# QEDProtocol/city-rollup

Measured on AMD Instinct MI355X. Metric: ms/NTT at 2^20 Goldilocks (commit-shaped step: 135-column 2^20-row NTT + Poseidon Merkle cap), lower is better.
Workload: dtype u64 (Goldilocks mod 2^64-2^32+1; the Poseidon MDS layers are evaluated exactly on 32-bit limbs held in f64); 1 GPU; configs[1]: 2^20-row x 135-column trace, forward NTT per column (natural->bit-reversed) + Poseidon Merkle cap height 4; log_n=20, columns=135, cap_height=4

## Files before the change

### city-rollup_amd/csrc/cityprover.hip

```cpp
#include "core.h"
#include "merkle.h"
#include "ntt.h"
#include "ntt16.h"
#include "poseidon.h"
#include "poseidon_coop.h"

namespace {

int get_pow_table(cp_ctx *ctx, uint64_t base, const uint64_t **out) {
  auto it = ctx->pow_tables.find(base);
  if (it != ctx->pow_tables.end()) {
    *out = it->second.get<uint64_t>();
    return CP_OK;
  }
  std::vector<uint64_t> h(3 * ntt::PT_SIZE);
  uint64_t b = base;
  for (int lvl = 0; lvl < 3; lvl++) {
    uint64_t acc = 1;
    for (int j = 0; j < ntt::PT_SIZE; j++) {
      h[lvl * ntt::PT_SIZE + j] = acc;
      acc = gl::mul(acc, b);
    }
    b = acc;
  }
  DevBuf t = ctx->buf();
  CP_TRY(alloc_status(ctx, t.alloc(h.size() * sizeof(uint64_t)), h.size() * sizeof(uint64_t)));
  HIP_TRY(ctx, hipMemcpyAsync(t.get(), h.data(), h.size() * sizeof(uint64_t), hipMemcpyHostToDevice, ctx->stream));
  HIP_TRY(ctx, hipStreamSynchronize(ctx->stream));
  *out = t.get<uint64_t>();
  ctx->pow_tables[base] = std::move(t);
  return CP_OK;
}

uint64_t root_of_unity(int log_n, bool inverse) {
  return inverse ? GL_ROOTS_INV[log_n] : GL_ROOTS[log_n];
}

int get_prescale_table(cp_ctx *ctx, int log_n, int rate_bits, uint64_t shift, const uint64_t **out) {
  cp_ctx::PreKey key{log_n, rate_bits, shift};
  auto it = ctx->prescale_tables.find(key);
  if (it != ctx->prescale_tables.end()) {
    *out = it->second.get<uint64_t>();
    return CP_OK;
  }
  const uint64_t *stab, *wtabN;
  CP_TRY(get_pow_table(ctx, shift, &stab));
  CP_TRY(get_pow_table(ctx, root_of_unity(log_n + rate_bits, false), &wtabN));
  size_t N = (size_t)1 << (log_n + rate_bits);
  DevBuf T = ctx->buf();
  CP_TRY(alloc_status(ctx, T.alloc(N * sizeof(uint64_t)), N * sizeof(uint64_t)));
  LAUNCH(ctx, "lde_fill_prescale", ntt16::k_fill_prescale, dim3((unsigned)((N + 255) / 256)), dim3(256), T.get<uint64_t>(),
         log_n, rate_bits, stab, wtabN);
  *out = T.get<uint64_t>();
  ctx->prescale_tables[key] = std::move(T);
  return CP_OK;
}

}
namespace quot {
__global__ __launch_bounds__(256) void k_fill_l0(uint64_t *out, size_t N, int log_N, int rb, const uint64_t *omega_tab, const uint64_t *zh,
                                                 uint64_t n_field);
}
namespace {

int get_l0_table(cp_ctx *ctx, int log_n, int rate_bits, const uint64_t *omega_tab, const uint64_t *zh, const uint64_t **out) {
  auto it = ctx->l0_tables.find({log_n, rate_bits});
  if (it == ctx->l0_tables.end()) {
    const size_t N = (size_t)1 << (log_n + rate_bits);
    DevBuf tab = ctx->buf();
    CP_TRY(alloc_status(ctx, tab.alloc(N * 8), N * 8));
    LAUNCH(ctx, "quotient_fill_l0", quot::k_fill_l0, dim3(blocks_for(N, 256)), dim3(256), tab.get<uint64_t>(), N, log_n + rate_bits, rate_bits,
           omega_tab, zh, ((uint64_t)1 << log_n) % gl::P);
    HIP_TRY(ctx, sync_stream(ctx));
    it = ctx->l0_tables.emplace(std::make_pair(log_n, rate_bits), std::move(tab)).first;
  }
  *out = it->second.get<uint64_t>();
  return CP_OK;
}

__global__ void k_self_test(const uint64_t *__restrict__ a, const uint64_t *__restrict__ b, uint64_t *__restrict__ out, int n_mul) {
  const int i = threadIdx.x;
  if (i < n_mul) out[i] = gl::mul(a[i], b[i]);
  if (i == 63) {
    uint64_t s[poseidon::W];
    for (int k = 0; k < poseidon::W; k++) s[k] = a[k];
    poseidon::permute(s);
    for (int k = 0; k < poseidon::W; k++) out[n_mul + k] = s[k];
  }
}
int power_on_self_test(cp_ctx *ctx) {
  constexpr int N = 16;
  const uint64_t M = ~0ull, P = gl::P;
  const uint64_t a[N] = {0, 1, P - 1, P - 1, M, M, 1ull << 48, 0xFFFFFFFFull << 32, 0x123456789ABCDEF1ull, 0xFFFFFFFF00000000ull,
                         0x8000000080000000ull, 0xFFFFFFFEFFFFFFFFull, 0xdeadbeefull << 32, 0x9E3779B97F4A7C15ull, 3, P + 5};
  const uint64_t b[N] = {M, M, P - 1, 2, M, P, 3ull << 48, 0xFFFFFFFFull << 32, 0xF0E1D2C3B4A59687ull, 0xFFFFFFFF00000001ull,
                         0x8000000080000000ull, 0xFFFFFFFEFFFFFFFFull, 0xfeedfaceull << 32, 0xD1B54A32D192ED03ull, M / 3, M - 7};
  uint64_t want[N + poseidon::W], got[N + poseidon::W];
  for (int i = 0; i < N; i++) want[i] = gl::mul(a[i], b[i]);
  {
    uint64_t s[poseidon::W];
    for (int k = 0; k < poseidon::W; k++) s[k] = a[k];
    poseidon::permute_host(s);
    for (int k = 0; k < poseidon::W; k++) want[N + k] = s[k];
  }
  CP_TRY(ensure_scratch(ctx, (3 * N + poseidon::W) * sizeof(uint64_t)));
  uint64_t *da = ctx->scratch.get<uint64_t>(), *db = da + N, *dout = db + N;
  CP_TRY(cp_h2d(ctx, da, a, sizeof a));
  CP_TRY(cp_h2d(ctx, db, b, sizeof b));
  LAUNCH(ctx, "self_test", k_self_test, dim3(1), dim3(64), da, db, dout, N);
  CP_TRY(cp_d2h(ctx, got, dout, sizeof got));
  if (hostu::fault_fires(CP_FAULT_SELFTEST)) got[7] ^= 1;
  for (int i = 0; i < N + poseidon::W; i++)
    if (got[i] != want[i])
      return set_error(ctx, CP_ERR_INTERNAL, "device arithmetic self-test failed (%s %d): this GPU does not execute the field kernels correctly",
                       i < N ? "product" : "permutation word", i < N ? i : i - N);
  return CP_OK;
}

int upload_constants(cp_ctx *ctx) {
  HIP_TRY(ctx, hipMemcpyToSymbol(HIP_SYMBOL(poseidon::d_RC), POSEIDON_RC, sizeof POSEIDON_RC));
  HIP_TRY(ctx, hipMemcpyToSymbol(HIP_SYMBOL(poseidon::d_RCD), POSEIDON_RCD, sizeof POSEIDON_RCD));
  HIP_TRY(ctx, hipMemcpyToSymbol(HIP_SYMBOL(poseidon::d_DDK), poseidon::DDK_HOST, sizeof poseidon::DDK_HOST));
  HIP_TRY(ctx, hipMemcpyToSymbol(HIP_SYMBOL(poseidon::d_DDLAST), poseidon::DDLAST_HOST, sizeof poseidon::DDLAST_HOST));
  return CP_OK;
}



struct DifExtra {
  const uint64_t *src = nullptr;
  size_t src_stride = 0;
  const uint64_t *ptab = nullptr;
  size_t block_stride = 0;
  int n_blocks = 1, block_bits = 0;
  bool natural_out = false;
};

int run_dif(cp_ctx *ctx, uint64_t *data, int log_n, size_t batch, size_t stride, bool inverse,
            uint64_t scale, const uint64_t *stab_pre, const DifExtra &ex = DifExtra()) {
  if (log_n == 0) return CP_OK;
  const uint64_t *wtab;
  CP_TRY(get_pow_table(ctx, root_of_unity(log_n, inverse), &wtab));
  int q = log_n;
  bool first = true;
  while (q > 0) {
    int L, c;
    int remaining = q;
    if (remaining <= ntt::LOG_TILE_MAX) {
      L = remaining;
    } else {
      int front = remaining - ntt::LOG_TILE_MAX;
      if (front >= 4 && front <= ntt::LOG_TILE_MAX - 4) L = front;
      else {
        int passes = (remaining + 9) / 10;
        L = (remaining + passes - 1) / passes;
      }
    }
    int q_after = q - L;
    c = ntt::LOG_TILE_MAX - L;
    int outer_bits = log_n - L;
    if (c > outer_bits) c = outer_bits;
    if (q_after > 0 && c > q_after) c = q_after;
    ntt::PassArgs a;
    a.data = data;
    a.stride = stride;
    a.wtab = wtab;
    a.stab = stab_pre;
    a.log_n = log_n;
    a.q = q_after;
    a.L = L;
    a.c = c;
    a.first = first;
    a.last = (q_after == 0);
    a.scale = scale;
    a.coset_pre = stab_pre != nullptr;
    a.coset_post = 0;
    a.src = ex.src;
    a.src_stride = ex.src_stride;
    a.ptab = ex.ptab;
    a.block_stride = ex.block_stride;
    a.block_bits = ex.block_bits;
    a.natural_out = ex.natural_out ? 1 : 0;
    const int staged = (int)CP_KNOB(ctx, "NTT_STAGED_STORE", 1);
    a.staged_store = (staged && q_after == 0 && log_n >= 16) ? 1 : 0;
    dim3 grid((unsigned)(((size_t)1 << outer_bits) >> c), (unsigned)batch, (unsigned)ex.n_blocks);
    bool done = false;
    const bool need16 = ex.src || ex.ptab || ex.n_blocks > 1 || ex.natural_out;
    static const bool ntt_v1 = getenv("CITYPROVER_NTT_V1") != nullptr;
    if (L >= 4 && L + c == ntt16::LOG_TILE && (need16 || !ntt_v1)) {
      const bool half = log_n >= 16;
#define PASS16_(LL, ROWS_, NAME)                                                                                              \
  if (inverse) {                                                                                                              \
    if (half) LAUNCH(ctx, NAME, (ntt16::k_dif_pass16<LL, 12 - LL, ROWS_, true, true>), grid, dim3(ntt16::THREADS), a);        \
    else LAUNCH(ctx, NAME, (ntt16::k_dif_pass16<LL, 12 - LL, ROWS_, true, false>), grid, dim3(ntt16::THREADS), a);            \
  } else {                                                                                                                    \
    if (half) LAUNCH(ctx, NAME, (ntt16::k_dif_pass16<LL, 12 - LL, ROWS_, false, true>), grid, dim3(ntt16::THREADS), a);       \
    else LAUNCH(ctx, NAME, (ntt16::k_dif_pass16<LL, 12 - LL, ROWS_, false, false>), grid, dim3(ntt16::THREADS), a);           \
  }
#define PASS16(LL)                                 \
  case LL:                                         \
    if (q_after == 0) {                            \
      PASS16_(LL, true, "ntt16_rows")              \
    } else {                                       \
      PASS16_(LL, false, "ntt16_cols")             \
    }                                              \
    done = true;                                   \
    break;
      switch (L) {
        PASS16(4) PASS16(5) PASS16(6) PASS16(7) PASS16(8) PASS16(9) PASS16(10) PASS16(11) PASS16(12)
        default: break;
      }
#undef PASS16
#undef PASS16_
    }
    if (!done && need16) return set_error(ctx, CP_ERR_INTERNAL, "radix-16 pass required but unavailable (L=%d c=%d)", L, c);
    if (!done) {
      if (q_after == 0)
        LAUNCH(ctx, "ntt_dif_pass_rows", ntt::k_dif_pass<true>, grid, dim3(ntt::THREADS), a);
      else
        LAUNCH(ctx, "ntt_dif_pass_cols", ntt::k_dif_pass<false>, grid, dim3(ntt::THREADS), a);
    }
    q = q_after;
    first = false;
  }
  return CP_OK;
}

int bitrev_copy(cp_ctx *ctx, const uint64_t *src, uint64_t *dst, size_t src_stride,
                size_t dst_stride, int log_n, size_t batch, const uint64_t *stab) {
  size_t n = (size_t)1 << log_n;
  dim3 grid(blocks_for(n, 256), (unsigned)batch);
  LAUNCH(ctx, "ntt_bitrev_copy", ntt::k_bitrev_copy, grid, dim3(256), src, dst, src_stride, dst_stride,
         log_n, stab);
  return CP_OK;
}

size_t merkle_words_per_tree(size_t n_leaves, int cap_height) {
  size_t cap_n = (size_t)1 << cap_height;
  size_t nodes = n_leaves > cap_n ? 2 * n_leaves - 2 * cap_n : n_leaves;
  return nodes * 4;
}

int merkle_fuse_levels(cp_ctx *ctx) {
  const int v = (int)CP_KNOB(ctx, "MERKLE_FUSE", 1);
  return v < 0 ? 0 : v > 3 ? 3 : v;
}
int merkle_level_fuse_levels(cp_ctx *ctx) {
  const int v = (int)CP_KNOB(ctx, "MERKLE_LEVEL_FUSE", 0);
  return v < 0 ? 0 : v > 3 ? 3 : v;
}
int fusable_levels(size_t nodes, size_t cap_n, int want) {
  if (nodes % merkle::THREADS) return 0;
  int f = 0;
  while (f < want && (nodes >> (f + 1)) > cap_n) f++;
  return f;
}

int merkle_levels(cp_ctx *ctx, uint64_t *D, size_t per_tree, size_t n_leaves, size_t n_trees,
                  int cap_height, uint64_t *caps, int done = 0) {
  size_t cap_n = (size_t)1 << cap_height;
  size_t n = n_leaves, off = 0;
  for (int l = 0; l < done; l++, n >>= 1) off += n * 4;
  while (n > cap_n) {
    size_t np = n / 2;
    const uint64_t *child = D + off;
    uint64_t *parent;
    size_t pstride;
    if (np == cap_n) { parent = caps; pstride = cap_n * 4; }
    else { parent = D + off + n * 4; pstride = per_tree; }
    const size_t coop_max = (size_t)CP_KNOB(ctx, "COOP_MAX", 16384);
    const int fuse_max = (int)CP_KNOB(ctx, "COOP_FUSE", pcoop::MAX_FUSED);
    if (np * n_trees <= coop_max && fuse_max >= 1) {
      while (n > cap_n) {
        int levels = 0;
        while (levels < fuse_max && levels < pcoop::MAX_FUSED && (n >> levels) > cap_n) levels++;
        const unsigned waves = ((1u << (levels - 1)) + pcoop::STATES_PER_WAVE - 1) / pcoop::STATES_PER_WAVE;
        LAUNCH(ctx, "merkle_levels_coop", pcoop::k_levels_coop, dim3((unsigned)(n >> levels), (unsigned)n_trees), dim3(64 * waves), D, off, n,
               levels, per_tree, caps, cap_n);
        for (int l = 0; l < levels; l++, n >>= 1) off += n * 4;
      }
      break;
    }
    int fuse = np == cap_n ? 0 : fusable_levels(np, cap_n, merkle_level_fuse_levels(ctx));
    while (fuse > 0 && (np >> fuse) * n_trees < coop_max) fuse--;
    if (fuse > 0) {
      const dim3 g((unsigned)(np / merkle::THREADS), (unsigned)n_trees), b(merkle::THREADS);
      if (fuse == 1) LAUNCH(ctx, "merkle_level_fused", merkle::k_level_fused<1>, g, b, D, off, np, per_tree);
      else if (fuse == 2) LAUNCH(ctx, "merkle_level_fused", merkle::k_level_fused<2>, g, b, D, off, np, per_tree);
      else LAUNCH(ctx, "merkle_level_fused", merkle::k_level_fused<3>, g, b, D, off, np, per_tree);
      for (int l = 0; l <= fuse; l++, n >>= 1) off += n * 4;
      continue;
    }
    if (np * n_trees <= coop_max)
      LAUNCH(ctx, "merkle_level_coop", pcoop::k_level_coop, dim3(blocks_for(np, pcoop::STATES_PER_BLOCK), (unsigned)n_trees), dim3(256), child,
             np, parent, per_tree, pstride);
    else
      LAUNCH(ctx, "merkle_level", merkle::k_level, dim3(blocks_for(np, merkle::THREADS), (unsigned)n_trees),
             dim3(merkle::THREADS), child, np, parent, per_tree, pstride);
    off += n * 4;
    n = np;
  }
  if (n_leaves == cap_n) {
    HIP_TRY(ctx, hipMemcpy2DAsync(caps, cap_n * 32, D, per_tree * 8, cap_n * 32, n_trees,
                                  hipMemcpyDeviceToDevice, ctx->stream));
  }
  return CP_OK;
}

int merkle_cols_batch(cp_ctx *ctx, const uint64_t *cols, size_t n_leaves, size_t leaf_len,
                      size_t col_stride, size_t n_trees, size_t tree_cols_stride, int cap_height,
                      uint64_t *digests, uint64_t *caps, const uint64_t *salt = nullptr, int n_salt = 0,
                      size_t salt_tree_stride = 0) {
  size_t per_tree = merkle_words_per_tree(n_leaves, cap_height);
  uint64_t *D = digests;
  if (!D) {
    CP_TRY(ensure_scratch(ctx, n_trees * per_tree * sizeof(uint64_t)));
    D = ctx->scratch.get<uint64_t>();
  }
  const dim3 grid(blocks_for(n_leaves, merkle::THREADS), (unsigned)n_trees), block(merkle::THREADS);
  const size_t coop_leaf_max = (size_t)CP_KNOB(ctx, "COOP_LEAF_MAX", 8192);
  const bool salted = salt && n_salt > 0;
  if (n_leaves * n_trees <= coop_leaf_max && leaf_len + (salted ? (size_t)n_salt : 0) > 4) {
    const dim3 cgrid(blocks_for(n_leaves, pcoop::STATES_PER_BLOCK), (unsigned)n_trees);
    if (salted)
      LAUNCH(ctx, "leaf_hash_cols_coop", pcoop::k_leaf_hash_cols_coop<true>, cgrid, dim3(256), cols, n_leaves, (int)leaf_len, col_stride, D,
             tree_cols_stride, per_tree, salt, n_salt, salt_tree_stride);
    else
      LAUNCH(ctx, "leaf_hash_cols_coop", pcoop::k_leaf_hash_cols_coop<false>, cgrid, dim3(256), cols, n_leaves, (int)leaf_len, col_stride, D,
             tree_cols_stride, per_tree, (const uint64_t *)nullptr, 0, (size_t)0);
    return merkle_levels(ctx, D, per_tree, n_leaves, n_trees, cap_height, caps);
  }
  const size_t coop_max = (size_t)CP_KNOB(ctx, "COOP_MAX", 16384);
  int fuse = fusable_levels(n_leaves, (size_t)1 << cap_height, merkle_fuse_levels(ctx));
  while (fuse > 0 && (n_leaves >> fuse) * n_trees < coop_max) fuse--;
#define CP_LEAF_LAUNCH(SALTED, F, SP, NS, SS)                                                                                          \
  LAUNCH(ctx, "leaf_hash_cols", (merkle::k_leaf_hash_cols<SALTED, F>), grid, block, cols, n_leaves, (int)leaf_len, col_stride, D, \
         tree_cols_stride, per_tree, SP, NS, SS)
  if (salted) {
    if (fuse == 3) CP_LEAF_LAUNCH(true, 3, salt, n_salt, salt_tree_stride);
    else if (fuse == 2) CP_LEAF_LAUNCH(true, 2, salt, n_salt, salt_tree_stride);
    else if (fuse == 1) CP_LEAF_LAUNCH(true, 1, salt, n_salt, salt_tree_stride);
    else CP_LEAF_LAUNCH(true, 0, salt, n_salt, salt_tree_stride);
  } else {
    if (fuse == 3) CP_LEAF_LAUNCH(false, 3, (const uint64_t *)nullptr, 0, (size_t)0);
    else if (fuse == 2) CP_LEAF_LAUNCH(false, 2, (const uint64_t *)nullptr, 0, (size_t)0);
    else if (fuse == 1) CP_LEAF_LAUNCH(false, 1, (const uint64_t *)nullptr, 0, (size_t)0);
    else CP_LEAF_LAUNCH(false, 0, (const uint64_t *)nullptr, 0, (size_t)0);
  }
#undef CP_LEAF_LAUNCH
  return merkle_levels(ctx, D, per_tree, n_leaves, n_trees, cap_height, caps, fuse);
}

bool valid_merkle_shape(size_t n_leaves, int cap_height) {
  if (n_leaves == 0 || (n_leaves & (n_leaves - 1))) return false;
  if (cap_height < 0 || cap_height > 40) return false;
  return ((size_t)1 << cap_height) <= n_leaves;
}

}

namespace { void batches_orphan(cp_ctx *ctx); }

extern "C" {

int cp_abi_version(void) { return CP_ABI_VERSION; }

int cp_fault_inject(int kind, long after) {
  if (kind != CP_FAULT_THREAD && kind != CP_FAULT_ALLOC && kind != CP_FAULT_SELFTEST && kind != CP_FAULT_DEVMEM) return set_error(nullptr, CP_ERR_INVALID_ARG, "unknown fault kind %d", kind);
  hostu::fault_counter(kind).store(after < 0 ? -1 : after);
  return CP_OK;
}

int cp_device_count(void) {
  int n = 0;
  if (hipGetDeviceCount(&n) != hipSuccess) return 0;
  return n;
}

const char *cp_last_error(cp_ctx *ctx) { return ctx ? ctx->error.c_str() : g_tls_error.c_str(); }

cp_ctx *cp_ctx_create(int device) try {
  int n = cp_device_count();
  if (n <= 0) {
    set_error(nullptr, CP_ERR_NO_DEVICE,
              "no HIP device visible: libcityprover_hip has no CPU fallback");
    return nullptr;
  }
  if (device < 0 || device >= n) {
    set_error(nullptr, CP_ERR_INVALID_ARG, "device %d out of range (have %d)", device, n);
    return nullptr;
  }
  cp_ctx *ctx = new (std::nothrow) cp_ctx(device);
  if (!ctx) {
    set_error(nullptr, CP_ERR_OOM, "out of host memory");
    return nullptr;
  }
  auto fail = [&](const char *what, hipError_t e) {
    set_error(nullptr, CP_ERR_HIP, "%s: %s", what, hipGetErrorString(e));
    delete ctx;
    return (cp_ctx *)nullptr;
  };
  hipError_t e = hipSetDevice(device);
  if (e != hipSuccess) return fail("hipSetDevice", e);
  e = hipStreamCreateWithFlags(&ctx->stream, hipStreamNonBlocking);
  if (e != hipSuccess) return fail("hipStreamCreate", e);
  if (upload_constants(ctx) != CP_OK || power_on_self_test(ctx) != CP_OK) {
    std::string msg = ctx->error;
    cp_ctx_destroy(ctx);
    g_tls_error = msg;
    return nullptr;
  }
  return ctx;
} catch (...) {
  exception_status(nullptr);
  return nullptr;
}

void cp_ctx_destroy(cp_ctx *ctx) {
  if (!ctx) return;
  batches_orphan(ctx);
  for (cp_ctx *lane : ctx->lanes) cp_ctx_destroy(lane);
  ctx->lanes.clear();
  hipSetDevice(ctx->device);
  if (ctx->stream) hipStreamSynchronize(ctx->stream);
  prof_flush(ctx);
  for (auto e : ctx->prof_pool) hipEventDestroy(e);
  ctx->pow_tables.clear(); ctx->prescale_tables.clear(); ctx->l0_tables.clear(); ctx->air_sel_tables.clear(); ctx->fr_twiddles.clear();
  ctx->arena.chunks.clear();
  for (DevBuf *b : {&ctx->scratch, &ctx->wires_stage, &ctx->fr_work, &ctx->fr_pow[0].tab, &ctx->fr_pow[1].tab, &ctx->msm_ws,
                     &ctx->fixed_base[0].tab, &ctx->fixed_base[1].tab}) b->reset();
  ctx->pin.reset();
  ctx->noncanonical_flag.reset();
  if (ctx->stream) hipStreamDestroy(ctx->stream);
  delete ctx;
}

int cp_ctx_set_lanes(cp_ctx *ctx, int lanes) try {
  CHECK_CTX(ctx);
  if (ctx->parent) return set_error(ctx, CP_ERR_INVALID_ARG, "a lane has no lanes of its own");
  if (lanes < 1 || lanes > 8) return set_error(ctx, CP_ERR_INVALID_ARG, "lanes must be 1..8 (got %d)", lanes);
  while ((int)ctx->lanes.size() < lanes) {
    cp_ctx *lane = cp_ctx_create(ctx->device);
    if (!lane) return lane_error(ctx);
    lane->parent = ctx;
    lane->transcript_mode = ctx->transcript_mode;
    ctx->lanes.push_back(lane);
  }
  ctx->n_lanes = lanes;
  return CP_OK;
} CP_CATCH(ctx)

int cp_ctx_set_option(cp_ctx *ctx, const char *name, long value) try {
  CHECK_CTX(ctx);
  if (!name) return set_error(ctx, CP_ERR_INVALID_ARG, "NULL argument");
  if (ctx->parent) return set_error(ctx, CP_ERR_INVALID_ARG, "a lane takes its options from its parent");
  bool known = false;
  for (const char *const *k = knob_names(); *k; k++) known = known || strcmp(*k, name) == 0;
  if (!known) return set_error(ctx, CP_ERR_INVALID_ARG, "unknown option \"%s\" (see INTEGRATION.md section 5b)", name);
  for (auto &kv : ctx->options)
    if (kv.first == name) { kv.second = value; return CP_OK; }
  ctx->options.emplace_back(name, value);
  return CP_OK;
} CP_CATCH(ctx)

int cp_ctx_set_device_transcript(cp_ctx *ctx, int mode) try {
  CHECK_CTX(ctx);
  if (mode < -1 || mode > 1) return set_error(ctx, CP_ERR_INVALID_ARG, "mode must be -1 (automatic), 0 (host) or 1 (device)");
  ctx->transcript_mode = mode;
  for (cp_ctx *l : ctx->lanes) l->transcript_mode = mode;
  return CP_OK;
} CP_CATCH(ctx)

int cp_dev_alloc(cp_ctx *ctx, size_t bytes, void **out) try {
  CHECK_CTX(ctx);
  if (!out) return set_error(ctx, CP_ERR_INVALID_ARG, "out is NULL");
  *out = nullptr;
  if (bytes == 0) return CP_OK;
  DevBuf b = ctx->buf();
  CP_TRY(alloc_status(ctx, b.alloc(bytes), bytes));
  *out = b.release();
  return CP_OK;
} CP_CATCH(ctx)
int cp_dev_free(cp_ctx *ctx, void *ptr) try {
  CHECK_CTX(ctx);
  if (!ptr) return CP_OK;
  HIP_TRY(ctx, hipStreamSynchronize(ctx->stream));
  HIP_TRY(ctx, abi_dev_free(ptr));
  return CP_OK;
} CP_CATCH(ctx)
int cp_host_alloc(cp_ctx *ctx, size_t bytes, void **out) try {
  CHECK_CTX(ctx);
  if (!out) return set_error(ctx, CP_ERR_INVALID_ARG, "out is NULL");
  *out = nullptr;
  if (bytes == 0) return CP_OK;
  PinBuf b(pin_pool(), ctx->device);
  CP_TRY(alloc_status(ctx, b.alloc(bytes), bytes));
  *out = b.release();
  return CP_OK;
} CP_CATCH(ctx)
int cp_host_free(cp_ctx *ctx, void *ptr) try {
  CHECK_CTX(ctx);
  if (!ptr) return CP_OK;
  HIP_TRY(ctx, hipStreamSynchronize(ctx->stream));
  HIP_TRY(ctx, abi_host_free(ptr));
  return CP_OK;
} CP_CATCH(ctx)
int cp_h2d(cp_ctx *ctx, void *dst, const void *src, size_t bytes) try {
  CHECK_CTX(ctx);
  if (bytes == 0) return CP_OK;
  if (!dst || !src) return set_error(ctx, CP_ERR_INVALID_ARG, "NULL pointer");
  HIP_TRY(ctx, hipMemcpyAsync(dst, src, bytes, hipMemcpyHostToDevice, ctx->stream));
// ... 422 lines not shown
```

### city-rollup_amd/csrc/ntt.h

```cpp
#pragma once
#include "gl.h"

namespace ntt {

constexpr int LOG_TILE_MAX = 12;
constexpr int TILE_MAX = 1 << LOG_TILE_MAX;
constexpr int THREADS = 256;
constexpr int PT_BITS = 11;
constexpr int PT_SIZE = 1 << PT_BITS;

__device__ __forceinline__ uint64_t pow_table(const uint64_t *__restrict__ T, uint64_t e) {
  uint32_t e0 = (uint32_t)e & (PT_SIZE - 1), e1 = (uint32_t)(e >> PT_BITS) & (PT_SIZE - 1),
           e2 = (uint32_t)(e >> (2 * PT_BITS));
  uint64_t r = T[e0];
  if (e1) r = gl::mul(r, T[PT_SIZE + e1]);
  if (e2) r = gl::mul(r, T[2 * PT_SIZE + e2]);
  return r;
}

__device__ __forceinline__ uint32_t bitrev(uint32_t x, int bits) {
  return bits ? (__brev(x) >> (32 - bits)) : 0;
}

struct PassArgs {
  uint64_t *data;
  size_t stride;
  const uint64_t *wtab;
  const uint64_t *stab;
  int log_n;
  int q, L, c;
  int first, last;
  uint64_t scale;
  int coset_pre;
  int coset_post;
  const uint64_t *src;
  size_t src_stride;
  const uint64_t *ptab;
  size_t block_stride;
  int block_bits;
  int natural_out;
  int staged_store;
};

template <bool ROWS_CONTIG>
__device__ __forceinline__ int lds_pos(int r, int cc, int L, int c) {
  return ROWS_CONTIG ? (cc << L) + r : (r << c) + cc;
}

template <bool ROWS_CONTIG>
__global__ __launch_bounds__(THREADS) void k_dif_pass(PassArgs a) {
  __shared__ uint64_t tile[TILE_MAX];
  __shared__ uint64_t ltw[TILE_MAX / 2];
  const int L = a.L, c = a.c, q = a.q;
  const int tile_elems = 1 << (L + c);
  const int tid = threadIdx.x;
  uint64_t *poly = a.data + (size_t)blockIdx.y * a.stride;
  const uint32_t o_base = blockIdx.x << c;
  const uint32_t qmask = (1u << q) - 1;

  for (int e = tid; e < (1 << (L - 1)); e += THREADS)
    ltw[e] = pow_table(a.wtab, (uint64_t)e << (a.log_n - L));

  for (int p = tid; p < tile_elems; p += THREADS) {
    int r, cc;
    if (ROWS_CONTIG) { cc = p >> L; r = p & ((1 << L) - 1); }
    else { r = p >> c; cc = p & ((1 << c) - 1); }
    uint32_t o = o_base + cc;
    size_t idx = ((size_t)(o >> q) << (q + L)) | ((size_t)r << q) | (o & qmask);
    uint64_t v = poly[idx];
    if (a.coset_pre && a.first) v = gl::mul(v, pow_table(a.stab, idx));
    tile[p] = v;
  }
  __syncthreads();

  const int n_bfly = tile_elems >> 1;
  for (int t = 0; t < L; t++) {
    const int hb = L - 1 - t;
    const int half = 1 << hb;
    for (int b = tid; b < n_bfly; b += THREADS) {
      int cc, pr;
      if (ROWS_CONTIG) { cc = b >> (L - 1); pr = b & ((1 << (L - 1)) - 1); }
      else { pr = b >> c; cc = b & ((1 << c) - 1); }
      int j = pr & (half - 1);
      int r0 = ((pr >> hb) << (hb + 1)) | j;
      int p0 = lds_pos<ROWS_CONTIG>(r0, cc, L, c), p1 = lds_pos<ROWS_CONTIG>(r0 + half, cc, L, c);
      uint64_t u = tile[p0], v = tile[p1];
      tile[p0] = gl::add(u, v);
      tile[p1] = gl::mul(gl::sub(u, v), ltw[j << t]);
    }
    __syncthreads();
  }

  for (int p = tid; p < tile_elems; p += THREADS) {
    int r, cc;
    if (ROWS_CONTIG) { cc = p >> L; r = p & ((1 << L) - 1); }
    else { r = p >> c; cc = p & ((1 << c) - 1); }
    uint32_t o = o_base + cc;
    uint32_t lo = o & qmask;
    size_t idx = ((size_t)(o >> q) << (q + L)) | ((size_t)r << q) | lo;
    uint64_t v = tile[p];
    if (q > 0) {
      uint64_t e = (uint64_t)lo * bitrev(r, L);
      if (e) v = gl::mul(v, pow_table(a.wtab, e << (a.log_n - q - L)));
    }
    if (a.last && a.scale) v = gl::mul(v, a.scale);
    poly[idx] = v;
  }
}

__global__ void k_bitrev_copy(const uint64_t *__restrict__ src, uint64_t *__restrict__ dst,
                              size_t src_stride, size_t dst_stride, int log_n,
                              const uint64_t *__restrict__ stab) {
  size_t i = (size_t)blockIdx.x * blockDim.x + threadIdx.x;
  if (i >> log_n) return;
  const uint64_t *s = src + (size_t)blockIdx.y * src_stride;
  uint64_t *d = dst + (size_t)blockIdx.y * dst_stride;
  uint64_t v = s[bitrev((uint32_t)i, log_n)];
  if (stab) v = gl::mul(v, pow_table(stab, i));
  d[i] = v;
}

__global__ void k_pad_copy(const uint64_t *__restrict__ src, uint64_t *__restrict__ dst,
                           size_t src_stride, size_t dst_stride, size_t n, size_t N) {
  size_t i = (size_t)blockIdx.x * blockDim.x + threadIdx.x;
  if (i >= N) return;
  dst[(size_t)blockIdx.y * dst_stride + i] = i < n ? src[(size_t)blockIdx.y * src_stride + i] : 0;
}

}
```

### city-rollup_amd/csrc/ntt16.h

```cpp
#pragma once
#include <type_traits>

#include "gl.h"
#include "ntt.h"

namespace ntt16 {

template <int K>
GL_HD uint64_t mul_pow2(uint64_t x) {
  static_assert(K >= 0 && K < 96, "shift out of range");
  if constexpr (K == 0) {
    return x;
  } else if constexpr (K < 64) {
    return gl::reduce128(x << K, x >> (64 - K));
  } else {
    constexpr int J = K - 64;
    uint64_t y0 = J ? (x << J) : x;
    uint64_t y1 = J ? (x >> (64 - J)) : 0;
    uint64_t t = gl::reduce128(0, y0);
    return gl::sub(t, y1 << 32);
  }
}

template <bool INV, int E>
GL_HD uint64_t diff_times_w16(uint64_t u, uint64_t v) {
  constexpr int SH = ((INV ? 36 : 156) * (E & 15)) % 192;
  constexpr bool NEG = SH >= 96;
  constexpr int K = SH % 96;
  uint64_t d = NEG ? gl::sub(v, u) : gl::sub(u, v);
  return mul_pow2<K>(d);
}

template <bool INV, int B, bool UNIT_T>
GL_HD void stage(uint64_t (&x)[16], uint64_t T) {
#pragma unroll
  for (int m = 0; m < 16; m++) {
    if (m & (1 << B)) continue;
    const int i = m & ((1 << B) - 1);
    uint64_t u = x[m], v = x[m + (1 << B)];
    x[m] = gl::add(u, v);
    uint64_t d;
    switch (i << (3 - B)) {
      case 0: d = diff_times_w16<INV, 0>(u, v); break;
      case 1: d = diff_times_w16<INV, 1>(u, v); break;
      case 2: d = diff_times_w16<INV, 2>(u, v); break;
      case 3: d = diff_times_w16<INV, 3>(u, v); break;
      case 4: d = diff_times_w16<INV, 4>(u, v); break;
      case 5: d = diff_times_w16<INV, 5>(u, v); break;
      case 6: d = diff_times_w16<INV, 6>(u, v); break;
      default: d = diff_times_w16<INV, 7>(u, v); break;
    }
    x[m + (1 << B)] = UNIT_T ? d : gl::mul(d, T);
  }
}

#if defined(NTT16_SINGLE_CHAINS) || defined(NTT16_STAGE_TWIDDLES)
#define NTT16_PAIRS 0
#else
#define NTT16_PAIRS 1
#endif

template <int K0, int K1>
GL_HD void mul_pow2_2(uint64_t &x, uint64_t &y) {
  static_assert(K0 > 0 && K0 < 96 && K1 > 0 && K1 < 96 && (K0 < 64) == (K1 < 64), "two shifts of one form");
  if constexpr (K0 < 64) {
    gl::reduce128_2(x << K0, x >> (64 - K0), y << K1, y >> (64 - K1), x, y);
  } else {
    constexpr int J0 = K0 - 64, J1 = K1 - 64;
    const uint64_t x0 = J0 ? (x << J0) : x, x1 = J0 ? (x >> (64 - J0)) : 0;
    const uint64_t y0 = J1 ? (y << J1) : y, y1 = J1 ? (y >> (64 - J1)) : 0;
    uint64_t t, u;
    gl::reduce128_2(0, x0, 0, y0, t, u);
    x = gl::sub(t, x1 << 32);
    y = gl::sub(u, y1 << 32);
  }
}

template <bool INV>
constexpr int w16_shift(int E) { return ((INV ? 36 : 156) * (E & 15)) % 192; }

struct ShiftPlan {
  int a[8], b[8], n;
};
template <bool INV, int B>
constexpr ShiftPlan shift_plan() {
  ShiftPlan p{};
  int pend[2] = {-1, -1};
  for (int m = 0; m < 16; m++) {
    if (m & (1 << B)) continue;
    const int K = w16_shift<INV>((m & ((1 << B) - 1)) << (3 - B)) % 96;
    if (K == 0) continue;
    const int form = K >= 64, reg = m + (1 << B);
    if (pend[form] < 0) {
      pend[form] = reg;
    } else {
      p.a[p.n] = pend[form];
      p.b[p.n++] = reg;
      pend[form] = -1;
    }
  }
  for (int form = 0; form < 2; form++)
    if (pend[form] >= 0) {
      p.a[p.n] = pend[form];
      p.b[p.n++] = -1;
    }
  return p;
}
template <bool INV, int B>
constexpr int reg_shift(int reg) { return w16_shift<INV>((reg & ((1 << B) - 1)) << (3 - B)) % 96; }

template <bool INV, int B, int I = 0>
GL_HD void apply_shifts(uint64_t (&x)[16]) {
  constexpr ShiftPlan p = shift_plan<INV, B>();
  if constexpr (I < p.n) {
    constexpr int ra = p.a[I], rb = p.b[I];
    if constexpr (rb < 0) x[ra] = mul_pow2<reg_shift<INV, B>(ra)>(x[ra]);
    else mul_pow2_2<reg_shift<INV, B>(ra), reg_shift<INV, B>(rb)>(x[ra], x[rb]);
    apply_shifts<INV, B, I + 1>(x);
  }
}

template <bool INV, int B>
GL_HD void stage_pairs(uint64_t (&x)[16]) {
#pragma unroll
  for (int m = 0; m < 16; m++) {
    if (m & (1 << B)) continue;
    const bool neg = w16_shift<INV>((m & ((1 << B) - 1)) << (3 - B)) >= 96;
    const uint64_t u = x[m], v = x[m + (1 << B)];
    x[m] = gl::add(u, v);
    x[m + (1 << B)] = neg ? gl::sub(v, u) : gl::sub(u, v);
  }
  apply_shifts<INV, B>(x);
}

constexpr int round_exp(int NSTAGES, int m) {
  int em = 0;
  for (int B = 3; B >= 4 - NSTAGES; B--) em += ((m >> B) & 1) << (3 - B);
  return em;
}
constexpr int round_reg(int NSTAGES, int E, int K) {
  for (int m = 0; m < 16; m++)
    if (round_exp(NSTAGES, m) == E && K-- == 0) return m;
  return -1;
}
template <int NSTAGES, int E, int K>
GL_HD void apply_power(uint64_t (&x)[16], uint64_t pw) {
  constexpr int CNT = 16 >> NSTAGES;
  if constexpr (K + 1 < CNT) {
    constexpr int m0 = round_reg(NSTAGES, E, K), m1 = round_reg(NSTAGES, E, K + 1);
    gl::mul2(x[m0], pw, x[m1], pw, x[m0], x[m1]);
    apply_power<NSTAGES, E, K + 2>(x, pw);
  } else if constexpr (K < CNT) {
    constexpr int m0 = round_reg(NSTAGES, E, K);
    x[m0] = gl::mul(x[m0], pw);
  }
}
template <int NSTAGES, int E = 1>
GL_HD void walk_powers(uint64_t (&x)[16], uint64_t pw, uint64_t T3) {
  constexpr int LAST = (1 << NSTAGES) - 1;
  if constexpr (E < LAST) {
    constexpr int m0 = round_reg(NSTAGES, E, 0);
    uint64_t next, r;
    gl::mul_lazy2(pw, T3, x[m0], pw, next, r);
    x[m0] = gl::canon(r);
    apply_power<NSTAGES, E, 1>(x, pw);
    walk_powers<NSTAGES, E + 1>(x, next, T3);
  } else {
    apply_power<NSTAGES, E, 0>(x, pw);
  }
}

template <bool INV, int NSTAGES, bool UNIT_T>
GL_HD void round16(uint64_t (&x)[16], uint64_t T3) {
#if defined(NTT16_STAGE_TWIDDLES)
  uint64_t T2 = UNIT_T ? 1 : gl::sqr(T3);
  stage<INV, 3, UNIT_T>(x, T3);
  if constexpr (NSTAGES >= 2) {
    stage<INV, 2, UNIT_T>(x, T2);
  }
  if constexpr (NSTAGES >= 3) {
    uint64_t T1 = UNIT_T ? 1 : gl::sqr(T2);
    stage<INV, 1, UNIT_T>(x, T1);
    if constexpr (NSTAGES >= 4) {
      uint64_t T0 = UNIT_T ? 1 : gl::sqr(T1);
      stage<INV, 0, UNIT_T>(x, T0);
    }
  }
#elif NTT16_PAIRS
  stage_pairs<INV, 3>(x);
  if constexpr (NSTAGES >= 2) stage_pairs<INV, 2>(x);
  if constexpr (NSTAGES >= 3) stage_pairs<INV, 1>(x);
  if constexpr (NSTAGES >= 4) stage_pairs<INV, 0>(x);
  if constexpr (!UNIT_T) walk_powers<NSTAGES>(x, T3, T3);
#else
  stage<INV, 3, true>(x, 1);
  if constexpr (NSTAGES >= 2) stage<INV, 2, true>(x, 1);
  if constexpr (NSTAGES >= 3) stage<INV, 1, true>(x, 1);
  if constexpr (NSTAGES >= 4) stage<INV, 0, true>(x, 1);
  if constexpr (!UNIT_T) {
    uint64_t pw = T3;
#pragma unroll
    for (int e = 1; e < (1 << NSTAGES); e++) {
      if (e > 1) pw = gl::mul_lazy(pw, T3);
#pragma unroll
      for (int m = 0; m < 16; m++) {
        int em = 0;
        for (int B = 3; B >= 4 - NSTAGES; B--) em += ((m >> B) & 1) << (3 - B);
        if (em == e) x[m] = gl::mul(x[m], pw);
      }
    }
  }
#endif
}

constexpr int LOG_TILE = 12;
constexpr int THREADS = 1 << (LOG_TILE - 4);

__device__ __forceinline__ int pad(int p) { return p + (p >> 4); }

template <bool HALF, typename T>
__device__ __forceinline__ void exchange(T *tile, uint64_t (&x)[16], int Pw, int Fw, int Pr, int Fr) {
  T *w = tile + pad(Pw), *r = tile + pad(Pr);
  if constexpr (HALF) {
    uint32_t lo[16];
#pragma unroll
    for (int m = 0; m < 16; m++) w[pad(m << Fw)] = gl::lo32(x[m]);
    __syncthreads();
#pragma unroll
    for (int m = 0; m < 16; m++) lo[m] = r[pad(m << Fr)];
    __syncthreads();
#pragma unroll
    for (int m = 0; m < 16; m++) w[pad(m << Fw)] = gl::hi32(x[m]);
    __syncthreads();
#pragma unroll
    for (int m = 0; m < 16; m++) x[m] = gl::pack(lo[m], r[pad(m << Fr)]);
  } else {
#pragma unroll
    for (int m = 0; m < 16; m++) w[pad(m << Fw)] = x[m];
    __syncthreads();
#pragma unroll
    for (int m = 0; m < 16; m++) x[m] = r[pad(m << Fr)];
  }
}

template <int L, int C, bool ROWS>
__device__ __forceinline__ size_t gidx(int pos, uint32_t tile_id, int q) {
  if (ROWS) return ((size_t)tile_id << LOG_TILE) + pos;
  uint32_t r = pos >> C, o = (tile_id << C) + (pos & ((1 << C) - 1));
  return ((size_t)(o >> q) << (q + L)) | ((size_t)r << q) | (o & ((1u << q) - 1));
}

#ifndef NTT16_MIN_WAVES
#define NTT16_MIN_WAVES 5
#endif
template <int L, int C, bool ROWS, bool INV, bool HALF>
__global__ __launch_bounds__(THREADS, (HALF && !(L == 4 && !ROWS)) ? NTT16_MIN_WAVES : 1) void k_dif_pass16(ntt::PassArgs a) {
  static_assert(L + C == LOG_TILE && L >= 4, "tile shape");
  using tile_t = typename std::conditional<HALF, uint32_t, uint64_t>::type;
  __shared__ tile_t tile[(1 << LOG_TILE) + (1 << (LOG_TILE - 4))];
  constexpr int B0 = ((L - 1) % 4) + 1;
  constexpr int NROUNDS = 1 + (L - B0) / 4;
  const int t = threadIdx.x;
  const int q = a.q;
  uint64_t *poly = a.data + (size_t)blockIdx.y * a.stride + (size_t)blockIdx.z * a.block_stride;
  const uint64_t *in = (a.first && a.src) ? a.src + (size_t)blockIdx.y * a.src_stride : poly;
  const uint64_t *ptab =
      (a.first && a.ptab) ? a.ptab + ((size_t)ntt::bitrev(blockIdx.z, a.block_bits) << a.log_n) : nullptr;
  uint64_t x[16];

  {
    constexpr int f = L - 4;
    constexpr int F = ROWS ? f : C + f;
    const int P = ((t >> F) << (F + 4)) | (t & ((1 << F) - 1));
    const uint64_t *in_t = ROWS ? in + ((size_t)blockIdx.x << LOG_TILE) : in;
    const uint64_t *ptab_t = (ROWS && ptab) ? ptab + ((size_t)blockIdx.x << LOG_TILE) : ptab;
#if !NTT16_PAIRS
#pragma unroll
    for (int m = 0; m < 16; m++) {
      const size_t idx = gidx<L, C, ROWS>(P + (m << F), blockIdx.x, q);
      uint64_t v = ROWS ? in_t[P + (m << F)] : in[idx];
      if (ptab) v = gl::mul(v, ROWS ? ptab_t[P + (m << F)] : ptab[idx]);
      else if (a.coset_pre && a.first) v = gl::mul(v, ntt::pow_table(a.stab, idx));
      x[m] = v;
    }
#else
#pragma unroll
    for (int m = 0; m < 16; m += 2) {
      const int p0 = P + (m << F), p1 = P + ((m + 1) << F);
      const size_t idx0 = gidx<L, C, ROWS>(p0, blockIdx.x, q), idx1 = gidx<L, C, ROWS>(p1, blockIdx.x, q);
      uint64_t v0 = ROWS ? in_t[p0] : in[idx0], v1 = ROWS ? in_t[p1] : in[idx1];
      if (ptab) gl::mul2(v0, ROWS ? ptab_t[p0] : ptab[idx0], v1, ROWS ? ptab_t[p1] : ptab[idx1], v0, v1);
      else if (a.coset_pre && a.first) gl::mul2(v0, ntt::pow_table(a.stab, idx0), v1, ntt::pow_table(a.stab, idx1), v0, v1);
      x[m] = v0;
      x[m + 1] = v1;
    }
#endif
    if constexpr (f == 0) {
      round16<INV, B0, true>(x, 1);
    } else {
      const int r = ROWS ? (P & ((1 << L) - 1)) : (P >> C);
      const uint32_t r_lo = r & ((1 << f) - 1);
      uint64_t T3 = ntt::pow_table(a.wtab, (uint64_t)r_lo << (a.log_n - f - 4));
      round16<INV, B0, false>(x, T3);
    }
  }
  constexpr int Flast = ROWS ? 0 : C;
  constexpr int F0 = ROWS ? (L - 4) : C + (L - 4);
  int Plast = ((t >> F0) << (F0 + 4)) | (t & ((1 << F0) - 1));
  int Fprev = F0;
#pragma unroll
  for (int k = 1; k < NROUNDS; k++) {
    const int f = L - B0 - 4 * k;
    const int F = ROWS ? f : C + f;
    const int P = ((t >> F) << (F + 4)) | (t & ((1 << F) - 1));
    exchange<HALF>(tile, x, Plast, Fprev, P, F);
    if (f == 0) {
      round16<INV, 4, true>(x, 1);
    } else {
      const int r = ROWS ? (P & ((1 << L) - 1)) : (P >> C);
      const uint32_t r_lo = r & ((1 << f) - 1);
      uint64_t T3 = ntt::pow_table(a.wtab, (uint64_t)r_lo << (a.log_n - f - 4));
      round16<INV, 4, false>(x, T3);
    }
    Plast = P;
    Fprev = F;
  }
  {
    const int P = Plast;
    if (!ROWS && q > 0) {
      const uint32_t cc = P & ((1 << C) - 1);
      const uint32_t r_base = P >> C;
      const uint32_t o = (blockIdx.x << C) + cc;
      const uint32_t lo = o & ((1u << q) - 1);
      if (lo) {
        const int sh = a.log_n - q - L;
        uint64_t W0 = ntt::pow_table(a.wtab, ((uint64_t)lo * ntt::bitrev(r_base, L)) << sh);
        uint64_t G = ntt::pow_table(a.wtab, ((uint64_t)lo << (L - 4)) << sh);
        uint64_t w = W0;
#pragma unroll
        for (int j = 0; j < 16; j++) {
          const int m = ((j & 1) << 3) | ((j & 2) << 1) | ((j & 4) >> 1) | ((j & 8) >> 3);
#if NTT16_PAIRS
          if (j < 15) {
            uint64_t r, next;
            gl::mul_lazy2(x[m], w, w, G, r, next);
            x[m] = gl::canon(r);
            w = next;
          } else {
            x[m] = gl::mul(x[m], w);
          }
#else
          x[m] = gl::mul(x[m], w);
          if (j < 15) w = gl::mul_lazy(w, G);
#endif
        }
      }
    }
    if (a.last && a.scale) {
#if NTT16_PAIRS
#pragma unroll
      for (int m = 0; m < 16; m += 2) gl::mul2(x[m], a.scale, x[m + 1], a.scale, x[m], x[m + 1]);
#else
#pragma unroll
      for (int m = 0; m < 16; m++) x[m] = gl::mul(x[m], a.scale);
#endif
    }
    if (ROWS && a.natural_out) {
      __syncthreads();
      if constexpr (HALF) {
        uint32_t lo[16];
#pragma unroll
        for (int m = 0; m < 16; m++) tile[pad((int)ntt::bitrev((uint32_t)(P + m), L))] = gl::lo32(x[m]);
        __syncthreads();
#pragma unroll
        for (int m = 0; m < 16; m++) lo[m] = tile[pad(t + (m << (LOG_TILE - 4)))];
        __syncthreads();
#pragma unroll
        for (int m = 0; m < 16; m++) tile[pad((int)ntt::bitrev((uint32_t)(P + m), L))] = gl::hi32(x[m]);
        __syncthreads();
#pragma unroll
        for (int m = 0; m < 16; m++) {
          int pos = t + (m << (LOG_TILE - 4));
          poly[((size_t)blockIdx.x << LOG_TILE) + pos] = gl::pack(lo[m], tile[pad(pos)]);
        }
      } else {
#pragma unroll
        for (int m = 0; m < 16; m++) tile[pad((int)ntt::bitrev((uint32_t)(P + m), L))] = x[m];
        __syncthreads();
#pragma unroll
        for (int m = 0; m < 16; m++) {
          int pos = t + (m << (LOG_TILE - 4));
          poly[((size_t)blockIdx.x << LOG_TILE) + pos] = tile[pad(pos)];
        }
      }
      return;
    }
    if (ROWS && a.staged_store) {
      uint64_t *out_t = poly + ((size_t)blockIdx.x << LOG_TILE);
      __syncthreads();
      if constexpr (HALF) {
        uint32_t lo[16];
        tile_t *w = tile + pad(P);
#pragma unroll
        for (int m = 0; m < 16; m++) w[pad(m)] = gl::lo32(x[m]);
        __syncthreads();
#pragma unroll
        for (int m = 0; m < 16; m++) lo[m] = tile[pad(t + (m << (LOG_TILE - 4)))];
        __syncthreads();
#pragma unroll
        for (int m = 0; m < 16; m++) w[pad(m)] = gl::hi32(x[m]);
        __syncthreads();
#pragma unroll
        for (int m = 0; m < 16; m++) {
          const int pos = t + (m << (LOG_TILE - 4));
          out_t[pos] = gl::pack(lo[m], tile[pad(pos)]);
        }
      } else {
        tile_t *w = tile + pad(P);
#pragma unroll
        for (int m = 0; m < 16; m++) w[pad(m)] = x[m];
        __syncthreads();
#pragma unroll
        for (int m = 0; m < 16; m++) {
          const int pos = t + (m << (LOG_TILE - 4));
          out_t[pos] = tile[pad(pos)];
        }
      }
    } else if (ROWS) {
      uint64_t *out_t = poly + ((size_t)blockIdx.x << LOG_TILE) + P;
#pragma unroll
      for (int m = 0; m < 16; m++) out_t[m << Flast] = x[m];
    } else {
#pragma unroll
      for (int m = 0; m < 16; m++) poly[gidx<L, C, ROWS>(P + (m << Flast), blockIdx.x, q)] = x[m];
    }
  }
}

__global__ void k_fill_prescale(uint64_t *__restrict__ T, int log_n, int rate_bits,
                                const uint64_t *__restrict__ stab, const uint64_t *__restrict__ wtabN) {
  size_t i = (size_t)blockIdx.x * blockDim.x + threadIdx.x;
  if (i >> (log_n + rate_bits)) return;
  uint64_t j = i & (((size_t)1 << log_n) - 1), r = i >> log_n;
  T[i] = gl::mul(ntt::pow_table(stab, j), ntt::pow_table(wtabN, (r * j) & (((uint64_t)1 << (log_n + rate_bits)) - 1)));
}

}
```

Baseline: 0.04841 ms/NTT.

## Process two NTT columns per block in the final radix-16 row pass

Adds a two-column variant of the radix-16 row pass: each block loads and transforms two columns at once, interleaving butterflies and twiddle multiplies across both register sets, and holds lo/hi halves in a doubled shared tile so each exchange needs fewer barriers. The aim is to share twiddle computation and raise instruction-level parallelism per thread. The cost is higher register and LDS use, with launch bounds lowered to 4 waves, so occupancy drops. It is enabled by default for the last row pass when there are at least two columns.

```diff
diff --git a/city-rollup_amd/csrc/cityprover.hip b/city-rollup_amd/csrc/cityprover.hip
--- a/city-rollup_amd/csrc/cityprover.hip
+++ b/city-rollup_amd/csrc/cityprover.hip
@@ -181,6 +181,7 @@
     a.block_stride = ex.block_stride;
     a.block_bits = ex.block_bits;
     a.natural_out = ex.natural_out ? 1 : 0;
+    a.batch = (int)batch;
     const int staged = (int)CP_KNOB(ctx, "NTT_STAGED_STORE", 1);
     a.staged_store = (staged && q_after == 0 && log_n >= 16) ? 1 : 0;
     dim3 grid((unsigned)(((size_t)1 << outer_bits) >> c), (unsigned)batch, (unsigned)ex.n_blocks);
@@ -189,6 +190,13 @@
     static const bool ntt_v1 = getenv("CITYPROVER_NTT_V1") != nullptr;
     if (L >= 4 && L + c == ntt16::LOG_TILE && (need16 || !ntt_v1)) {
       const bool half = log_n >= 16;
+      const long pair_columns = CP_KNOB(ctx, "NTT_PAIR_COLUMNS", ntt16::PAIR_COLUMNS_DEFAULT);
+      if (half && batch >= 2 && !need16 && log_n <= 28 && q_after == 0 && L == 12 && (pair_columns & 2)) {
+        grid.y = (unsigned)((batch + 1) / 2);
+        if (inverse) LAUNCH(ctx, "ntt16_rows", (ntt16::k_dif_pass16<12, 0, true, true, true, 2>), grid, dim3(ntt16::THREADS), a);
+        else LAUNCH(ctx, "ntt16_rows", (ntt16::k_dif_pass16<12, 0, true, false, true, 2>), grid, dim3(ntt16::THREADS), a);
+        done = true;
+      }
 #define PASS16_(LL, ROWS_, NAME)                                                                                              \
   if (inverse) {                                                                                                              \
     if (half) LAUNCH(ctx, NAME, (ntt16::k_dif_pass16<LL, 12 - LL, ROWS_, true, true>), grid, dim3(ntt16::THREADS), a);        \
@@ -206,7 +214,7 @@
     }                                              \
     done = true;                                   \
     break;
-      switch (L) {
+      if (!done) switch (L) {
         PASS16(4) PASS16(5) PASS16(6) PASS16(7) PASS16(8) PASS16(9) PASS16(10) PASS16(11) PASS16(12)
         default: break;
       }
diff --git a/city-rollup_amd/csrc/ntt.h b/city-rollup_amd/csrc/ntt.h
--- a/city-rollup_amd/csrc/ntt.h
+++ b/city-rollup_amd/csrc/ntt.h
@@ -40,6 +40,7 @@
   int block_bits;
   int natural_out;
   int staged_store;
+  int batch;
 };
 
 template <bool ROWS_CONTIG>
diff --git a/city-rollup_amd/csrc/ntt16.h b/city-rollup_amd/csrc/ntt16.h
--- a/city-rollup_amd/csrc/ntt16.h
+++ b/city-rollup_amd/csrc/ntt16.h
@@ -213,6 +213,76 @@
 #endif
 }
 
+template <bool INV, int B, int I = 0>
+GL_HD void apply_shifts(uint64_t (&x)[2][16]) {
+  constexpr ShiftPlan p = shift_plan<INV, B>();
+  if constexpr (I < p.n) {
+    constexpr int ra = p.a[I], rb = p.b[I], Ka = reg_shift<INV, B>(ra);
+    if constexpr (rb < 0) {
+      mul_pow2_2<Ka, Ka>(x[0][ra], x[1][ra]);
+    } else {
+      mul_pow2_2<Ka, reg_shift<INV, B>(rb)>(x[0][ra], x[0][rb]);
+      mul_pow2_2<Ka, reg_shift<INV, B>(rb)>(x[1][ra], x[1][rb]);
+    }
+    apply_shifts<INV, B, I + 1>(x);
+  }
+}
+GL_HD void settle(uint64_t &s, uint64_t &d) {
+#if GL_DEVICE_ASM
+  asm volatile("" : "+v"(s), "+v"(d));
+#endif
+}
+template <bool INV, int B>
+GL_HD void stage_pairs(uint64_t (&x)[2][16]) {
+#pragma unroll
+  for (int c = 0; c < 2; c++) {
+#pragma unroll
+    for (int m = 0; m < 16; m++) {
+      if (m & (1 << B)) continue;
+      const bool neg = w16_shift<INV>((m & ((1 << B) - 1)) << (3 - B)) >= 96;
+      const uint64_t u = x[c][m], v = x[c][m + (1 << B)];
+      x[c][m] = gl::add(u, v);
+      x[c][m + (1 << B)] = neg ? gl::sub(v, u) : gl::sub(u, v);
+      settle(x[c][m], x[c][m + (1 << B)]);
+    }
+  }
+  apply_shifts<INV, B>(x);
+}
+template <int NSTAGES, int E, int K>
+GL_HD void apply_power(uint64_t (&x)[2][16], uint64_t pw) {
+  if constexpr (K < (16 >> NSTAGES)) {
+    constexpr int m = round_reg(NSTAGES, E, K);
+    gl::mul2(x[0][m], pw, x[1][m], pw, x[0][m], x[1][m]);
+    apply_power<NSTAGES, E, K + 1>(x, pw);
+  }
+}
+template <int NSTAGES, int E = 1>
+GL_HD void walk_powers(uint64_t (&x)[2][16], uint64_t pw, uint64_t T3) {
+  constexpr int LAST = (1 << NSTAGES) - 1;
+  if constexpr (E < LAST) {
+    constexpr int m0 = round_reg(NSTAGES, E, 0);
+    uint64_t p1, p2, r0, r1;
+    gl::mul_lazy2(pw, T3, x[0][m0], pw, p1, r0);
+    gl::mul_lazy2(p1, T3, x[1][m0], pw, p2, r1);
+    x[0][m0] = gl::canon(r0);
+    x[1][m0] = gl::canon(r1);
+    apply_power<NSTAGES, E, 1>(x, pw);
+    apply_power<NSTAGES, E + 1, 0>(x, p1);
+    walk_powers<NSTAGES, E + 2>(x, p2, T3);
+  } else {
+    static_assert(E == LAST, "odd exponents end on the last");
+    apply_power<NSTAGES, E, 0>(x, pw);
+  }
+}
+template <bool INV, int NSTAGES, bool UNIT_T>
+GL_HD void round16(uint64_t (&x)[2][16], uint64_t T3) {
+  stage_pairs<INV, 3>(x);
+  if constexpr (NSTAGES >= 2) stage_pairs<INV, 2>(x);
+  if constexpr (NSTAGES >= 3) stage_pairs<INV, 1>(x);
+  if constexpr (NSTAGES >= 4) stage_pairs<INV, 0>(x);
+  if constexpr (!UNIT_T) walk_powers<NSTAGES>(x, T3, T3);
+}
+
 constexpr int LOG_TILE = 12;
 constexpr int THREADS = 1 << (LOG_TILE - 4);
 
@@ -250,14 +320,127 @@
   return ((size_t)(o >> q) << (q + L)) | ((size_t)r << q) | (o & ((1u << q) - 1));
 }
 
+constexpr int TILE_WORDS = (1 << LOG_TILE) + (1 << (LOG_TILE - 4));
+constexpr long PAIR_COLUMNS_DEFAULT = 2;
+
+__device__ __forceinline__ int tile_pos(int t, int F) { return ((t >> F) << (F + 4)) | (t & ((1 << F) - 1)); }
+
+template <int Fw, int Fr>
+__device__ __forceinline__ void exchange(uint32_t (&tile)[2][TILE_WORDS], uint64_t (&x)[2][16], int t) {
+  uint32_t *w = tile[0] + pad(tile_pos(t, Fw)), *r = tile[0] + pad(tile_pos(t, Fr));
+#pragma unroll
+  for (int c = 0; c < 2; c++) {
+    if (c) __syncthreads();
+#pragma unroll
+    for (int m = 0; m < 16; m++) {
+      w[pad(m << Fw)] = gl::lo32(x[c][m]);
+      w[TILE_WORDS + pad(m << Fw)] = gl::hi32(x[c][m]);
+    }
+    __syncthreads();
+#pragma unroll
+    for (int m = 0; m < 16; m++) x[c][m] = gl::pack(r[pad(m << Fr)], r[TILE_WORDS + pad(m << Fr)]);
+  }
+}
+
+__device__ __forceinline__ void from_here(uint32_t &v) { asm volatile("" : "+v"(v)); }
+__device__ __forceinline__ uint64_t &at_bytes(uint64_t *base, uint32_t off) { return *(uint64_t *)((char *)base + off); }
+
+template <int L, bool INV, int K>
+__device__ __forceinline__ void later_rounds(const ntt::PassArgs &a, uint32_t (&tile)[2][TILE_WORDS], uint64_t (&x)[2][16], int t) {
+  constexpr int B0 = ((L - 1) % 4) + 1;
+  if constexpr (K < 1 + (L - B0) / 4) {
+    constexpr int f = L - B0 - 4 * K, fprev = K == 1 ? L - 4 : f + 4;
+    exchange<fprev, f>(tile, x, t);
+    if constexpr (f == 0) {
+      round16<INV, 4, true>(x, 1);
+    } else {
+      uint32_t r_lo = tile_pos(t, f) & ((1 << f) - 1);
+      from_here(r_lo);
+      round16<INV, 4, false>(x, ntt::pow_table(a.wtab, (uint64_t)r_lo << (a.log_n - f - 4)));
+    }
+    later_rounds<L, INV, K + 1>(a, tile, x, t);
+  }
+}
+
+template <int L, bool INV>
+__device__ __forceinline__ void pass16_two_columns(const ntt::PassArgs &a, uint32_t (&tile)[2][TILE_WORDS]) {
+  constexpr int B0 = ((L - 1) % 4) + 1;
+  const int t = threadIdx.x;
+  const bool two = 2 * blockIdx.y + 1 < (uint32_t)a.batch;
+  uint64_t *const col0 = a.data + (size_t)(2 * blockIdx.y) * a.stride, *const col1 = col0 + a.stride;
+  uint64_t x[2][16];
+
+  {
+    constexpr int f = L - 4;
+    const int P = tile_pos(t, f);
+    const uint32_t off0 = ((blockIdx.x << LOG_TILE) + P) << 3, step = 8u << f;
+#pragma unroll
+    for (int m = 0; m < 16; m++) x[0][m] = at_bytes(col0, off0 + m * step);
+    if (two) {
+#pragma unroll
+      for (int m = 0; m < 16; m++) x[1][m] = at_bytes(col1, off0 + m * step);
+    } else {
+#pragma unroll
+      for (int m = 0; m < 16; m++) x[1][m] = 0;
+    }
+    if constexpr (f == 0) {
+      round16<INV, B0, true>(x, 1);
+    } else {
+      const uint32_t r_lo = P & ((1 << f) - 1);
+      round16<INV, B0, false>(x, ntt::pow_table(a.wtab, (uint64_t)r_lo << (a.log_n - f - 4)));
+    }
+  }
+  later_rounds<L, INV, 1>(a, tile, x, t);
+  uint32_t te = threadIdx.x;
+  from_here(te);
+  const int P = tile_pos((int)te, 0);
+  if (a.last && a.scale) {
+#pragma unroll
+    for (int m = 0; m < 16; m++) gl::mul2(x[0][m], a.scale, x[1][m], a.scale, x[0][m], x[1][m]);
+  }
+  if (a.staged_store) {
+    uint32_t *w = tile[0] + pad(P);
+    const uint32_t *r = tile[0] + pad((int)te);
+    const uint32_t off0 = ((blockIdx.x << LOG_TILE) + te) << 3;
+#pragma unroll
+    for (int c = 0; c < 2; c++) {
+      if (c && !two) break;
+      __syncthreads();
+#pragma unroll
+      for (int m = 0; m < 16; m++) {
+        w[pad(m)] = gl::lo32(x[c][m]);
+        w[TILE_WORDS + pad(m)] = gl::hi32(x[c][m]);
+      }
+      __syncthreads();
+#pragma unroll
+      for (int m = 0; m < 16; m++)
+        at_bytes(c ? col1 : col0, off0 + (m << (LOG_TILE - 4 + 3))) = gl::pack(r[m * 272], r[TILE_WORDS + m * 272]);
+    }
+  } else {
+    const uint32_t off0 = ((blockIdx.x << LOG_TILE) + P) << 3;
+#pragma unroll
+    for (int m = 0; m < 16; m++) at_bytes(col0, off0 + 8 * m) = x[0][m];
+    if (two) {
+#pragma unroll
+      for (int m = 0; m < 16; m++) at_bytes(col1, off0 + 8 * m) = x[1][m];
+    }
+  }
+}
+
 #ifndef NTT16_MIN_WAVES
 #define NTT16_MIN_WAVES 5
 #endif
-template <int L, int C, bool ROWS, bool INV, bool HALF>
-__global__ __launch_bounds__(THREADS, (HALF && !(L == 4 && !ROWS)) ? NTT16_MIN_WAVES : 1) void k_dif_pass16(ntt::PassArgs a) {
+template <int L, int C, bool ROWS, bool INV, bool HALF, int NCOL = 1>
+__global__ __launch_bounds__(THREADS, NCOL == 2 ? 4 : (HALF && !(L == 4 && !ROWS)) ? NTT16_MIN_WAVES : 1) void k_dif_pass16(ntt::PassArgs a) {
   static_assert(L + C == LOG_TILE && L >= 4, "tile shape");
+  static_assert(NCOL == 1 || (NCOL == 2 && HALF && ROWS && L >= 5), "two columns: row passes, half-tile exchange, at least two rounds");
   using tile_t = typename std::conditional<HALF, uint32_t, uint64_t>::type;
-  __shared__ tile_t tile[(1 << LOG_TILE) + (1 << (LOG_TILE - 4))];
+  __shared__ tile_t tiles[NCOL][TILE_WORDS];
+  if constexpr (NCOL == 2) {
+    pass16_two_columns<L, INV>(a, tiles);
+    return;
+  }
+  tile_t(&tile)[TILE_WORDS] = tiles[0];
   constexpr int B0 = ((L - 1) % 4) + 1;
   constexpr int NROUNDS = 1 + (L - B0) / 4;
   const int t = threadIdx.x;
```

New measurement: 0.04811 ms/NTT, median of 6. About the same (-0.6%).
